# ctu-vras/depth_correction

Measured on AMD Instinct MI355X. Metric: points/sec through min_eigval_loss fwd+bwd (200k pts, k=10); HBM GB/s vs peak, higher is better.
Workload: dtype f64

## Files before the change

### depth_correction_amd/csrc/dc_cons_chain.h

```cpp
#pragma once

namespace dc {

struct AdamArgs {
  double* p; double* m; double* v;
  int n;
  double grad_scale, lr, b1, b2, eps, weight_decay, bias1, bias2_sqrt;
};
__device__ __forceinline__ void adam_apply(const AdamArgs& a, int i, double grad, double p0, double m0, double v0) {
  double g = grad * a.grad_scale;
  if (a.weight_decay != 0.0) g += a.weight_decay * p0;
  const double mi = m0 + (g - m0) * (1.0 - a.b1);
  const double vi = v0 * a.b2 + (1.0 - a.b2) * g * g;
  a.m[i] = mi; a.v[i] = vi;
  const double denom = sqrt(vi) / a.bias2_sqrt + a.eps;
  a.p[i] = p0 + (-(a.lr / a.bias1)) * (mi / denom);
}
__device__ __forceinline__ void adam_update(const AdamArgs& a, int i, double grad) { adam_apply(a, i, grad, a.p[i], a.m[i], a.v[i]); }

struct StepChain {
  int32_t* ready;
  uint32_t stamp;
  int parity, has_prev, n_front, n_out;
  int reverse;
  const double* prev;
  int64_t prev_rows;
  const double* grad_sum;
  double* out_prev;
  double* w_prev_out;
  int32_t* status;
  int spin_limit;
  const double* w_now;
  const int32_t* prev_status;
  const double* acc_in;
  AdamArgs adam;
  const uint8_t* blk_skip;
};
constexpr int32_t kStatusChainTimeout = 2;
constexpr int kChainFront = 8;

__device__ __forceinline__ int64_t chain_block_of(const StepChain& ch, bool chained, int64_t nblocks) {
  const int64_t b = (int64_t)blockIdx.x - (chained ? ch.n_front : 0);
  if (!(chained && ch.reverse)) return xcd_block_of(b, nblocks);
  const int64_t per = (nblocks + kXcds - 1) / kXcds;
  const int64_t logical = (b % kXcds) * per + (per - 1 - b / kXcds);
  return logical < nblocks ? logical : -1;
}

__device__ __forceinline__ void chain_publish(const StepChain& ch, int k, double w) {
  unsigned long long* pub = reinterpret_cast<unsigned long long*>(ch.ready);
  const unsigned long long st = (unsigned long long)ch.stamp << 32;
  __hip_atomic_store(pub + 2 * k, st | (unsigned)__double2loint(w), __ATOMIC_RELAXED, __HIP_MEMORY_SCOPE_AGENT);
  __hip_atomic_store(pub + 2 * k + 1, st | (unsigned)__double2hiint(w), __ATOMIC_RELAXED, __HIP_MEMORY_SCOPE_AGENT);
}

template <int P>
__device__ __forceinline__ void chain_front_block(const StepChain& ch, double* lds ) {
  const int a = blockIdx.x;
  if (a == 0 && ch.has_prev && !ch.grad_sum)
    for (int z = 2 + P + threadIdx.x; z < ch.n_out; z += kBlock) ch.out_prev[z] = 0.0;
  if (a >= 2 + P) return;
  if (ch.grad_sum) {
    if (a >= 2 && threadIdx.x == 0) {
      if (ch.has_prev && ch.adam.p) adam_update(ch.adam, a - 2, ch.grad_sum[a - 2]);
      const double wk = ch.adam.p ? ch.adam.p[a - 2] : ch.w_now[a - 2];
      chain_publish(ch, a - 2, wk);
      if (ch.w_prev_out) ch.w_prev_out[a - 2] = wk;
    }
    return;
  }
  const bool step = ch.has_prev && ch.adam.p && a >= 2 && threadIdx.x == 0;
  const int32_t* st_prev = ch.prev_status ? ch.prev_status : ch.status;
  const bool flagged = ch.has_prev && a == 0 && threadIdx.x == 0 && st_prev &&
                       __hip_atomic_load(st_prev, __ATOMIC_RELAXED, __HIP_MEMORY_SCOPE_AGENT) != 0;
  double p0 = 0.0, m0 = 0.0, v0 = 0.0;
  if (step) {
    p0 = ch.adam.p[a - 2]; m0 = ch.adam.m[a - 2]; v0 = ch.adam.v[a - 2];
    if (ch.w_prev_out) ch.w_prev_out[a - 2] = p0;
  }
  double s = 0.0;
  if (ch.has_prev) {
    const double* p = ch.prev + (int64_t)a * ch.prev_rows;
    constexpr int U = 32;
    for (int64_t r0 = threadIdx.x; r0 < ch.prev_rows; r0 += (int64_t)U * kBlock) {
      double v[U];
#pragma unroll
      for (int u_ = 0; u_ < U; ++u_) v[u_] = (r0 + (int64_t)u_ * kBlock < ch.prev_rows) ? p[r0 + (int64_t)u_ * kBlock] : 0.0;
#pragma unroll
      for (int w_ = U / 2; w_ > 0; w_ >>= 1) {
#pragma unroll
        for (int u_ = 0; u_ < w_; ++u_) v[u_] += v[u_ + w_];
      }
      s += v[0];
    }
    s = wave_sum(s);
  }
  const int lane = threadIdx.x & (kWave - 1), wave = threadIdx.x / kWave;
  if (lane == 0) lds[wave] = s;
  __syncthreads();
  if (threadIdx.x == 0) {
    if (ch.has_prev) {
      double t = 0.0;
      for (int wv = 0; wv < kBlock / kWave; ++wv) t += lds[wv];
      if (ch.acc_in) t += ch.acc_in[a];
      if (flagged) t = __longlong_as_double(0x7ff8000000000000ll);
      ch.out_prev[a] = t;
      if (step) adam_apply(ch.adam, a - 2, t, p0, m0, v0);
    }
    if (a >= 2) chain_publish(ch, a - 2, step ? ch.adam.p[a - 2] : ch.w_now[a - 2]);
  }
}

template <int P>
__global__ __launch_bounds__(kBlock) void chain_front_only_kernel(StepChain ch) {
  __shared__ double s_front[kBlock / kWave];
  chain_front_block<P>(ch, s_front);
}

template <int P>
__device__ __forceinline__ void chain_weights(const StepChain& ch, double w_scale, double* s_w, int* s_ok) {
  const int tid = threadIdx.x;
  if (tid == 0) *s_ok = 1;
  if (tid < 2 * P) {
    const unsigned long long* pub = reinterpret_cast<const unsigned long long*>(ch.ready) + tid;
    unsigned long long word = 0;
    bool ok = false;
    for (int spin = 0; spin < ch.spin_limit; ++spin) {
      word = __hip_atomic_load(pub, __ATOMIC_RELAXED, __HIP_MEMORY_SCOPE_AGENT);
      if ((uint32_t)(word >> 32) == ch.stamp) { ok = true; break; }
      __builtin_amdgcn_s_sleep(2);
    }
    const int half = (int)(uint32_t)word;
    const int other = __shfl_xor(half, 1, kWave);
    if ((tid & 1) == 0) s_w[tid >> 1] = (ok ? __hiloint2double(other, half) : __longlong_as_double(0x7ff8000000000000ll)) * w_scale;
    if (!ok) {
      *s_ok = 0;
      if (ch.status) atomicOr(ch.status, kStatusChainTimeout);
    }
  }
}

}
```

### depth_correction_amd/csrc/dc_cons_step.h

```cpp
#pragma once

namespace dc {

template <typename PT, int P> struct StepRow;
template <int P> struct StepRow<q32, P> {
  static constexpr int kPieces = (6 + P + 3) / 4;
  struct Raw { int32_t q[6 + P]; };
  static __device__ __forceinline__ Raw fetch(const PointBasis& pb, int64_t row) {
    const int32_t* r = static_cast<const int32_t*>(pb.rows) + row * (6 + P);
    Raw o;
#pragma unroll
    for (int c = 0; c < 6 + P; ++c) o.q[c] = r[c];
    return o;
  }
  static __device__ __forceinline__ void stage(const PointBasis& pb, const double* wq, int64_t row, int4* tile, int cap, int t) {
    place(fetch(pb, row), wq, tile, cap, t);
  }
  static __device__ __forceinline__ void place(const Raw& raw, const double* wq, int4* tile, int cap, int t) {
    const int32_t* q = raw.q;
    float sc = 0.0f;
#pragma unroll
    for (int k = 0; k < P; ++k) sc = fmaf((float)wq[k], __int_as_float(q[6 + k]), sc);
    int32_t x[3];
#pragma unroll
// ... 199 lines not shown
    for (int u_ = 0; u_ < kTrip; ++u_) nxt[u_] = (q0 + kTrip + u_ < nslots) ? (uint32_t)lrow[(q0 + kTrip + u_) * kBlock] : kNoLoc;
    float g[P];
#pragma unroll
    for (int k = 0; k < P; ++k) g[k] = 0.0f;
#pragma unroll
    for (int u_ = 0; u_ < kTrip; ++u_) chain_term_f32<P>(tile, cap, l[u_], l[u_] != kNoLoc, ci, cmf, vs, vu, c2f, g);
#pragma unroll
    for (int k = 0; k < P; ++k) gw[k] += (double)g[k];
  }
}
template <typename PT, int P>
__device__ __forceinline__ void chain_tail(const int4* tile, int cap, const uint16_t* lrow, int nslots, bool packed, const double* mean,
                                           const double* v0, double c1, double c2, double* gw) {
  uint32_t nxt[kTrip];
#pragma unroll
  for (int u_ = 0; u_ < kTrip; ++u_) nxt[u_] = (kPreSlots + u_ < nslots) ? (uint32_t)lrow[(kPreSlots + u_) * kBlock] : kNoLoc;
  for (int q0 = kPreSlots; q0 < nslots; q0 += kTrip) {
    uint32_t l[kTrip];
#pragma unroll
    for (int u_ = 0; u_ < kTrip; ++u_) l[u_] = nxt[u_];
    if (packed && __all((int)(l[0] == kNoLoc))) break;
#pragma unroll
    for (int u_ = 0; u_ < kTrip; ++u_) nxt[u_] = (q0 + kTrip + u_ < nslots) ? (uint32_t)lrow[(q0 + kTrip + u_) * kBlock] : kNoLoc;
#pragma unroll
    for (int u_ = 0; u_ < kTrip; ++u_) chain_term<PT, P>(tile, cap, l[u_], l[u_] != kNoLoc, mean, v0, c1, c2, gw);
  }
}

template <int CTRL>
__device__ __forceinline__ double dpp_f64(double v) {
  const int lo = __builtin_amdgcn_mov_dpp(__double2loint(v), CTRL, 0xF, 0xF, true);
  const int hi = __builtin_amdgcn_mov_dpp(__double2hiint(v), CTRL, 0xF, 0xF, true);
  return __hiloint2double(hi, lo);
}
constexpr int kDppXor1 = 0xB1;
constexpr int kDppXor2 = 0x4E;
constexpr int kDppRor4 = 0x124;
constexpr int kDppRor8 = 0x128;
constexpr int kDppShl4 = 0x104;
constexpr int kDppQuad3 = 0xFF;
__device__ __forceinline__ double wave_sum4_dpp(double* v) {
  const int lane = threadIdx.x & (kWave - 1);
  const bool up1 = (lane & 1) != 0, up2 = (lane & 2) != 0;
  const double k0 = up1 ? v[2] : v[0], g0 = up1 ? v[0] : v[2];
  const double k1 = up1 ? v[3] : v[1], g1 = up1 ? v[1] : v[3];
  const double a0 = k0 + dpp_f64<kDppXor1>(g0);
  const double a1 = k1 + dpp_f64<kDppXor1>(g1);
  const double kk = up2 ? a1 : a0, gg = up2 ? a0 : a1;
  double r = kk + dpp_f64<kDppXor2>(gg);
  r += dpp_f64<kDppRor4>(r);
  r += dpp_f64<kDppRor8>(r);
  r += __shfl_xor(r, 16, kWave);
  r += __shfl_xor(r, 32, kWave);
  return r;
}

template <int P, bool DPP = false>
__device__ __forceinline__ void step_partials(const double* acc2, const double* gw, double* __restrict__ p_fwd, double* __restrict__ p_bwd,
                                              bool per_block = false, int n_front = 0) {
  constexpr int NV = 2 + P, NP2 = NV <= 4 ? 4 : 8;
  __shared__ double s_comb[kWavesPerBlock][NP2];
  double v[NP2];
  v[0] = acc2[0]; v[1] = acc2[1];
#pragma unroll
  for (int k = 0; k < NP2 - 2; ++k) v[2 + k] = k < P ? gw[k] : 0.0;
  double tot;
  if constexpr (DPP && NP2 == 4) tot = wave_sum4_dpp(v);
  else tot = wave_sum_packed<NP2>(v);
  const int lane = threadIdx.x & (kWave - 1), wave = threadIdx.x / kWave;
  int64_t rs = (int64_t)gridDim.x * kWavesPerBlock, row = (int64_t)blockIdx.x * kWavesPerBlock + wave;
  if (per_block) {
    if (lane < NP2) s_comb[wave][lane] = tot;
    __syncthreads();
    if (wave != 0) return;
    if (lane < NP2) tot = (s_comb[0][lane] + s_comb[1][lane]) + (s_comb[2][lane] + s_comb[3][lane]);
    rs = (int64_t)gridDim.x - n_front;
    row = (int64_t)blockIdx.x - n_front;
  }
  if (lane < NP2) {
    const int q = packed_value_of_lane<NP2>(lane);
    if (q < 2) p_fwd[q * rs + row] = tot;
    else if (q < NV) p_bwd[(q - 2) * rs + row] = tot;
  }
}

template <typename PT, int NS, int P, int VAR = 0>
__global__ __launch_bounds__(kBlock) void consistency_step_basis_kernel(
    PointBasis pb, BlockTab tab, const int32_t* __restrict__ own_base, int cap, const int32_t* __restrict__ centre_idx, int64_t n,
    const uint8_t* __restrict__ mask, LossParams lp, QParams qp, double* __restrict__ p_fwd, double* __restrict__ p_bwd,
    StepChain ch) {
  extern __shared__ int4 tile[];
  __shared__ double s_w[DC_MAX_MODEL_TERMS];
  __shared__ int s_ok;
  __shared__ double s_front[kBlock / kWave];
  const bool chained = ch.ready != nullptr;
  if (chained && (int)blockIdx.x < ch.n_front) { chain_front_block<P>(ch, s_front); return; }
  const int64_t nblocks = (n + kBlock - 1) / kBlock;
  int64_t blk = chain_block_of(ch, chained, nblocks);
  if (blk >= 0 && ch.blk_skip && ch.blk_skip[blk]) blk = -1;
  double acc2[2] = {0.0, 0.0}, gw[P];
#pragma unroll
  for (int k = 0; k < P; ++k) gw[k] = 0.0;
  const int32_t s0 = blk >= 0 ? tab.slot_ptr[blk] : 0;
  bool bad = blk >= 0 && tab.slot_ptr[blk + 1] - s0 != NS;
  if (blk >= 0 && !bad) {
    const int64_t i = blk * kBlock + threadIdx.x;
// ... 64 lines not shown
            if (q % 4 == 0 && q > 0) __builtin_amdgcn_sched_barrier(0);
            chain_term_f32<P>(tile, cap, pre[q], true, ci, cmf, vs, vu, c2f, gwf);
          }
        }
#pragma unroll
        for (int k = 0; k < P; ++k) gw[k] = (double)gwf[k] * u;
      } else {
        double mean[3];
        StepRow<PT, P>::mean_of(ci, cm, mean);
        if (any_miss) {
#pragma unroll
          for (int q = 0; q < NS; ++q) chain_term<PT, P>(tile, cap, pre[q], pre[q] != kNoLoc, mean, v0, c1, c2, gw);
        } else {
#pragma unroll
          for (int q = 0; q < NS; ++q) chain_term<PT, P>(tile, cap, pre[q], true, mean, v0, c1, c2, gw);
        }
#pragma unroll
        for (int k = 0; k < P; ++k) gw[k] *= u;
      }
    }
  }
  if (bad) acc2[0] = acc2[1] = __longlong_as_double(0x7ff8000000000000ll);
  step_partials<P, (VAR & kVarDppSums) != 0>(acc2, gw, p_fwd, p_bwd, chained, chained ? ch.n_front : 0);
}

constexpr int kStepQ32Cap = 512;

typedef float float2v __attribute__((ext_vector_type(2)));
template <int P, int CAP>
__device__ __forceinline__ void chain_term_q32(const int4* tile, uint32_t off, bool have, const Pt<q32>::Raw& ci, const float* cmf, const float* vs,
                                               const float* vu, float c2f, float* gw) {
  const char* row = reinterpret_cast<const char*>(tile) + (have ? off : 0u);
  const int4 p0 = *reinterpret_cast<const int4*>(row);
  const int4 p1 = *reinterpret_cast<const int4*>(row + (size_t)CAP * 16);
  const float2v e01 = float2v{(float)(p0.x - ci.v[0]), (float)(p0.y - ci.v[1])} - float2v{cmf[0], cmf[1]};
  const float e0 = e01.x, e1 = e01.y, e2 = (float)(p0.z - ci.v[2]) - cmf[2];
  const float u0 = __int_as_float(p0.w), u1 = __int_as_float(p1.x), u2 = __int_as_float(p1.y);
  const float al = fmaf(vs[2], e2, fmaf(vs[1], e1, vs[0] * e0));
  const float be = fmaf(vu[2], u2, fmaf(vu[1], u1, vu[0] * u0));
  const float ga = fmaf(e2, u2, fmaf(e1, u1, e0 * u0));
  float tj = fmaf(al, be, -(c2f * ga));
  if (!have) tj = 0.0f;
  if constexpr (P == 2) {
    float2v g = float2v{gw[0], gw[1]};
    g = __builtin_elementwise_fma(float2v{tj, tj}, float2v{__int_as_float(p1.z), __int_as_float(p1.w)}, g);
    gw[0] = g.x; gw[1] = g.y;
  } else {
    gw[0] = fmaf(tj, __int_as_float(p1.z), gw[0]);
    if constexpr (P > 1) gw[1] = fmaf(tj, __int_as_float(p1.w), gw[1]);
    if constexpr (P > 2) gw[2] = fmaf(tj, __int_as_float(reinterpret_cast<const int4*>(row + (size_t)CAP * 32)->x), gw[2]);
  }
}

#ifdef DC_BLOCK_TRACE
__device__ unsigned long long* g_block_trace = nullptr;
#define DC_TRACE_BEGIN() const unsigned long long trace_t0 = __builtin_amdgcn_s_memrealtime()
#define DC_TRACE_END() do { if (threadIdx.x == 0 && g_block_trace) { \
    unsigned long long* tr_ = g_block_trace + 4 * (size_t)blockIdx.x; \
    tr_[0] = ((unsigned long long)__builtin_amdgcn_s_getreg((31 << 11) | 20) << 32) | (unsigned)__builtin_amdgcn_s_getreg((31 << 11) | 4); \
    tr_[1] = trace_t0; tr_[2] = __builtin_amdgcn_s_memrealtime(); tr_[3] = 1; } } while (0)
#else
#define DC_TRACE_BEGIN() do {} while (0)
#define DC_TRACE_END() do {} while (0)
#endif

template <int NS, int P, int CAP>
__global__ __launch_bounds__(kBlock, (StepRow<q32, P>::kPieces * CAP * 16 <= 25 * 1024 ? 6 : 4)) void consistency_step_q32_kernel(
    PointBasis pb, BlockTab tab, const int32_t* __restrict__ own_base, const int32_t* __restrict__ centre_idx, int64_t n,
    const uint8_t* __restrict__ mask, LossParams lp, QParams qp, double* __restrict__ p_fwd, double* __restrict__ p_bwd,
    StepChain ch) {
  constexpr int NV = 2 + P, NP2 = NV <= 4 ? 4 : 8;
  constexpr int cap = CAP;
  __shared__ int4 tile[StepRow<q32, P>::kPieces * CAP];
  __shared__ double s_w[DC_MAX_MODEL_TERMS];
  __shared__ double s_front[kWavesPerBlock];
  __shared__ double s_comb[kWavesPerBlock * NP2];
  __shared__ int s_ok[2];
  DC_TRACE_BEGIN();
  const bool chained = ch.ready != nullptr;
  if (chained && (int)blockIdx.x < ch.n_front) { chain_front_block<P>(ch, s_front); return; }
  const int64_t nblocks = (n + kBlock - 1) / kBlock;
  int64_t blk = chain_block_of(ch, chained, nblocks);
  if (blk >= 0 && ch.blk_skip && ch.blk_skip[blk]) blk = -1;
  double acc2[2] = {0.0, 0.0}, gw[P];
#pragma unroll
  for (int k = 0; k < P; ++k) gw[k] = 0.0;
  const int32_t s0 = blk >= 0 ? tab.slot_ptr[blk] : 0;
  bool bad = blk >= 0 && tab.slot_ptr[blk + 1] - s0 != NS;
  if (blk >= 0 && !bad) {
    const int64_t i = blk * kBlock + threadIdx.x;
    const bool live = i < n;
    const bool in_mask = live && (mask ? mask[i] != 0 : true);
    const uint16_t* lrow = tab.loc + (int64_t)s0 * kBlock + threadIdx.x;
    uint32_t pre[NS];
#pragma unroll
    for (int q = 0; q < NS; ++q) pre[q] = (uint32_t)lrow[q * kBlock];
    const int32_t base = tab.blk_ptr[blk], nd = tab.blk_ptr[blk + 1] - base;
    const int32_t own = (own_base && !centre_idx) ? own_base[blk] : -1;
    double wq[P];
    if (chained) {
      typename StepRow<q32, P>::Raw r0, r1;
      const int t0 = threadIdx.x, t1 = threadIdx.x + kBlock;
      if (t0 < nd) r0 = StepRow<q32, P>::fetch(pb, tab.blk_ids[base + t0]);
      if (t1 < nd) r1 = StepRow<q32, P>::fetch(pb, tab.blk_ids[base + t1]);
      chain_weights<P>(ch, pb.w_scale, s_w, s_ok);
      __syncthreads();
      if (!s_ok[0]) bad = true;
#pragma unroll
      for (int k = 0; k < P; ++k) wq[k] = s_w[k];
      if (t0 < nd) StepRow<q32, P>::place(r0, wq, tile, cap, t0);
      if (t1 < nd) StepRow<q32, P>::place(r1, wq, tile, cap, t1);
      for (int t = threadIdx.x + 2 * kBlock; t < nd; t += kBlock) StepRow<q32, P>::stage(pb, wq, tab.blk_ids[base + t], tile, cap, t);
    } else {
      stage_weights(pb, s_w);
      __syncthreads();
#pragma unroll
      for (int k = 0; k < P; ++k) wq[k] = s_w[k];
      for (int t = threadIdx.x; t < nd; t += kBlock) StepRow<q32, P>::stage(pb, wq, tab.blk_ids[base + t], tile, cap, t);
    }
    Pt<q32>::Raw ci;
    if (own < 0) ci = Basis<q32>::template point<P>(pb, wq, live ? (centre_idx ? (int64_t)centre_idx[i] : i) : 0);
    __syncthreads();
    if (own >= 0) ci = staged_point<q32>(tile, cap, own + (live ? (int)threadIdx.x : 0));
    if (live && (!mask || __any((int)in_mask))) {
      CovAcc acc;
      cov_init(acc);
      uint32_t mo = pre[0];
#pragma unroll
      for (int q = 1; q < NS; ++q) mo |= pre[q];
      const bool any_miss = __any((int)(mo & 1u)) != 0;
      int n_have;
      if (any_miss) n_have = gather_fixed<q32, NS, true>(tile, cap, ci, pre, acc);
      else n_have = gather_fixed<q32, NS, false>(tile, cap, ci, pre, acc);
      acc.W = (double)n_have;
      double cm[3], v0[3], c1, c2;
      step_point2<q32, NS>(acc, n_have, !any_miss, in_mask, lp, qp, acc2, cm, v0, &c1, &c2);
      float cmf[3], vs[3], vu[3], gwf[P];
#pragma unroll
      for (int a = 0; a < 3; ++a) { cmf[a] = (float)cm[a]; vs[a] = (float)(c1 * v0[a]); vu[a] = (float)v0[a]; }
      const float c2f = (float)c2;
#pragma unroll
      for (int k = 0; k < P; ++k) gwf[k] = 0.0f;
      if (any_miss) {
#pragma unroll
        for (int q = 0; q < NS; ++q) {
          if (q % 4 == 0 && q > 0) __builtin_amdgcn_sched_barrier(0);
          chain_term_q32<P, CAP>(tile, pre[q], pre[q] != kNoLoc, ci, cmf, vs, vu, c2f, gwf);
        }
      } else {
#pragma unroll
        for (int q = 0; q < NS; ++q) {
          if (q % 4 == 0 && q > 0) __builtin_amdgcn_sched_barrier(0);
          chain_term_q32<P, CAP>(tile, pre[q], true, ci, cmf, vs, vu, c2f, gwf);
        }
      }
      const double u = qp.scale;
#pragma unroll
      for (int k = 0; k < P; ++k) gw[k] = (double)gwf[k] * u;
    }
  }
  if (bad) acc2[0] = acc2[1] = __longlong_as_double(0x7ff8000000000000ll);
  double v[NP2];
  v[0] = acc2[0]; v[1] = acc2[1];
#pragma unroll
  for (int k = 0; k < NP2 - 2; ++k) v[2 + k] = k < P ? gw[k] : 0.0;
  double tot;
  if constexpr (NP2 == 4) tot = wave_sum4_dpp(v);
  else tot = wave_sum_packed<NP2>(v);
  const int lane = threadIdx.x & (kWave - 1), wave = threadIdx.x / kWave;
  int64_t rs = (int64_t)gridDim.x * kWavesPerBlock, row = (int64_t)blockIdx.x * kWavesPerBlock + wave;
  if (chained) {
    if (lane < NP2) s_comb[wave * NP2 + lane] = tot;
    __syncthreads();
    if (wave != 0) return;
    if (lane < NP2) tot = (s_comb[lane] + s_comb[NP2 + lane]) + (s_comb[2 * NP2 + lane] + s_comb[3 * NP2 + lane]);
    rs = (int64_t)gridDim.x - ch.n_front;
    row = (int64_t)blockIdx.x - ch.n_front;
  }
  if (lane < NP2) {
    const int q = packed_value_of_lane<NP2>(lane);
    if (q < 2) p_fwd[q * rs + row] = tot;
    else if (q < NV) p_bwd[(q - 2) * rs + row] = tot;
  }
  DC_TRACE_END();
}

template <typename PT, int P>
__global__ __launch_bounds__(kBlock) void consistency_step_basis_slots_kernel(
    PointBasis pb, BlockTab tab, const int32_t* __restrict__ own_base, int cap, const int32_t* __restrict__ centre_idx, int64_t n,
    const uint8_t* __restrict__ mask, LossParams lp, QParams qp, double* __restrict__ p_fwd, double* __restrict__ p_bwd,
    StepChain ch, int packed) {
  extern __shared__ int4 tile[];
  __shared__ double s_w[DC_MAX_MODEL_TERMS];
  __shared__ int s_ok;
  __shared__ double s_front[kBlock / kWave];
  const bool chained = ch.ready != nullptr;
  if (chained && (int)blockIdx.x < ch.n_front) { chain_front_block<P>(ch, s_front); return; }
  const int64_t nblocks = (n + kBlock - 1) / kBlock;
  int64_t blk = xcd_block_of((int64_t)blockIdx.x - (chained ? ch.n_front : 0), nblocks);
  if (blk >= 0 && ch.blk_skip && ch.blk_skip[blk]) blk = -1;
  double acc2[2] = {0.0, 0.0}, gw[P];
#pragma unroll
  for (int k = 0; k < P; ++k) gw[k] = 0.0;
  const int64_t i = blk * kBlock + threadIdx.x;
  const bool live = blk >= 0 && i < n;
  int32_t nslots = 0, own = -1, base = 0, nd = 0;
  const uint16_t* lrow = tab.loc;
  uint32_t pre[kPreSlots];
  if (blk >= 0) {
    const int32_t s0 = tab.slot_ptr[blk];
    nslots = tab.slot_ptr[blk + 1] - s0;
    lrow = tab.loc + (int64_t)s0 * kBlock + threadIdx.x;
#pragma unroll
    for (int q = 0; q < kPreSlots; ++q) pre[q] = (live && q < nslots) ? (uint32_t)lrow[q * kBlock] : kNoLoc;
    own = (own_base && !centre_idx) ? own_base[blk] : -1;
    base = tab.blk_ptr[blk];
    nd = tab.blk_ptr[blk + 1] - base;
  }
  double wq[P];
  bool timed_out = false;
  typename Pt<PT>::Raw ci;
  if (chained) {
// ... 222 lines not shown
```

### depth_correction_amd/csrc/dc_consistency.hip

```cpp
#include <type_traits>
#include <atomic>
#include <mutex>
#include <cstdio>
#include <hip/hip_ext.h>
#include "dc_common.h"
#include "dc_device.h"
#include "dc_pointmath.h"
#include "dc_prof.h"
#include "dc_points_dev.h"
#include "../../include/dc_hip.h"

namespace dc {

template <typename T, typename PT, int STRIDE>
__global__ __launch_bounds__(kBlock) void points_fwd_kernel(PointInputs in, int64_t n, QParams qp, PT* __restrict__ x_out,
                                                            T* __restrict__ vps_out, T* __restrict__ dirs_out,
                                                            T* __restrict__ depth_out) {
  __shared__ double s_pose[kLdsScans * 12];
  const int64_t i = (int64_t)blockIdx.x * kBlock + threadIdx.x;
  const int64_t ic = i < n ? i : n - 1;
  ModelParams mp;
  load_model(in, mp);
  T vp_r[3] = {T(0), T(0), T(0)}, dr_r[3];
  if (in.vps) { const T* q = (const T*)in.vps + ic * 3; vp_r[0] = q[0]; vp_r[1] = q[1]; vp_r[2] = q[2]; }
// ... 943 lines not shown
  const bool step = adam.p && a >= 2 && a - 2 < adam.n && threadIdx.x == 0;
  double p0 = 0.0, m0 = 0.0, v0 = 0.0;
  if (step) { p0 = adam.p[a - 2]; m0 = adam.m[a - 2]; v0 = adam.v[a - 2]; }
  const double s = wave_sum(strided_sum(p, n_rows));
  if (lane == 0) lds[wave] = s;
  __syncthreads();
  if (threadIdx.x == 0) {
    double t = 0.0;
    for (int wv = 0; wv < kRedBlock / kWave; ++wv) t += lds[wv];
    if (flagged) t = __longlong_as_double(0x7ff8000000000000ll);
    out[a] = t;
    if (step) adam_apply(adam, a - 2, t, p0, m0, v0);
  }
}

static inline unsigned red_grid(int n_red, int pose_first, int pose_cols) {
  if (pose_first < 0 || n_red <= pose_first) return 2u + (unsigned)n_red;
  return 2u + (unsigned)pose_first + (unsigned)((pose_cols + kPoseRedCols - 1) / kPoseRedCols);
}

__global__ void adam_kernel(const double* __restrict__ grad, AdamArgs adam) {
  const int i = (int)(blockIdx.x * blockDim.x + threadIdx.x);
  if (i < adam.n) adam_update(adam, i, grad[i]);
}

__global__ __launch_bounds__(256) void adam_device_step_kernel(const double* __restrict__ grad, AdamArgs adam, int64_t* __restrict__ step) {
  const double t = (double)(*step + 1);
  adam.bias1 = 1.0 - pow(adam.b1, t);
  adam.bias2_sqrt = sqrt(1.0 - pow(adam.b2, t));
  for (int i = threadIdx.x; i < adam.n; i += blockDim.x) adam_update(adam, i, grad[i]);
  __syncthreads();
  if (threadIdx.x == 0) *step = (int64_t)t;
}

}

using namespace dc;

#define DC_CHECK_LAUNCH()                                  \
  do {                                                     \
    hipError_t err__ = hipGetLastError();                  \
    if (err__ != hipSuccess) return (int)err__;            \
  } while (0)

static inline int64_t n_blocks(int64_t n) { return (n + kBlock - 1) / kBlock; }
static std::atomic<bool> g_no_tab{false};
static std::atomic<int> g_fwd_generic{0};
static std::atomic<bool> g_no_basis{false};
static std::atomic<bool> g_two_pass{false};
static std::atomic<int> g_chain_spin{1 << 22};
static std::atomic<int> g_step_var{1};
static std::atomic<bool> g_pose_three_pass{false};
static std::atomic<bool> g_no_reverse{false};

template <int P, int CAP>
static int ragged_launch(dim3 grid, hipStream_t stream, hipEvent_t ev0, hipEvent_t ev1, const PointBasis& pb, const BlockTab& tab,
                         const dcBlockTable* t, int64_t n_rows, const uint8_t* mask, const LossParams& lp, const QParams& qp, double* p_fwd,
                         double* p_bwd, const StepChain& ch) {
  constexpr size_t bytes = (size_t)StepRow<q32, P>::kPieces * CAP * 16;
  static std::atomic<uint64_t> attr_set{0};
  if (bytes > 60 * 1024) {
    int dev = 0;
    if (hipGetDevice(&dev) != hipSuccess) dev = 0;
    const uint64_t bit = 1ull << (dev & 63);
    if (!(attr_set.fetch_or(bit) & bit)) {
      hipError_t err = hipFuncSetAttribute((const void*)consistency_step_ragged_q32_kernel<P, CAP>, hipFuncAttributeMaxDynamicSharedMemorySize, (int)bytes);
      if (err != hipSuccess) { attr_set.fetch_and(~bit); return (int)err; }
    }
  }
  hipExtLaunchKernelGGL((consistency_step_ragged_q32_kernel<P, CAP>), grid, dim3(kBlock), bytes, stream, ev0, ev1, 0, pb, tab, t->own_base, t->row_ptr, n_rows,
                        mask, lp, qp, p_fwd, p_bwd, ch);
  return DC_OK;
}

static bool use_table(const dcBlockTable* t, int layout, int stride, uint32_t row_bytes, int extra_rows, size_t lds_limit,
                      size_t* lds_bytes, int* lds_rows) {
  if (!t || g_no_tab.load() || stride != 4 || t->layout != layout || !t->blk_ptr || !t->loc || t->max_rows < 0) return false;
  if (layout == DC_TABLE_SLOTS ? !t->slot_ptr : !t->run_ptr) return false;
  if (t->max_rows > 0 && !t->blk_ids) return false;
  const size_t rows = (size_t)t->max_rows + extra_rows + (t->max_rows + extra_rows == 0 ? 1 : 0);
  const size_t need = rows * row_bytes;
  if (need > lds_limit || t->max_rows >= 0xFFF) return false;
  *lds_bytes = need;
  *lds_rows = (int)rows;
  return true;
}

extern "C" {

int dc_version(void) { return 100; }

int64_t dc_partial_rows(int64_t n) { return xcd_grid(n_blocks(n)) * kWavesPerBlock; }

int dc_param_grad_count(int n_terms, int n_scans) { return 2 * n_terms + 12 * n_scans; }

int64_t dc_sequence_partials_count(int64_t n, int n_terms, int n_scans) {
  if (n < 0 || n_terms < 0 || n_scans < 0) return 0;
  const int64_t rows = xcd_grid(n_blocks(n)) * kWavesPerBlock;
  return rows * (2 + 2 * (int64_t)n_terms + 12 * (int64_t)n_scans) + 2 * (2 + (int64_t)n_terms) * rows;
}

static PointInputs make_inputs(const void* vps, const void* dirs, const void* depth, const void* inc,
                               const uint8_t* lmask, const int32_t* scan_id, const double* poses, int n_scans,
                               int model_kind, int n_terms, const double* w, const double* e) {
  PointInputs in;
  in.vps = vps; in.dirs = dirs; in.depth = depth; in.inc = inc; in.lmask = lmask; in.scan_id = scan_id;
// ... 295 lines not shown
  if (n < 0 || !grad_points || !dirs || !depth || !partials_ws || !grads_out || (stride != 3 && stride != 4))
    return DC_ERR_ARG;
  if (scan_id && (!poses || n_scans < 1)) return DC_ERR_ARG;
  int rc = check_model(model_kind, n_terms, inc, w, e);
  if (rc) return rc;
  if (model_kind == DC_MODEL_NONE) n_terms = 0;
  const int n_acc = 2 * n_terms + 12 * n_scans;
  if (n_acc == 0) return DC_OK;
  if (n == 0) return (int)hipMemsetAsync(grads_out, 0, n_acc * sizeof(double), stream);
  PointInputs in = make_inputs(vps, dirs, depth, inc, lmask, scan_id, poses, n_scans, model_kind, n_terms, w, e);
  const int64_t rows = n_blocks(n);
  const int64_t prows = rows * kWavesPerBlock;
  dim3 grid((unsigned)rows), block(kBlock);
  const int n_red = want_pose_grad ? n_acc : 2 * n_terms;
  if (n_red < n_acc) {
    hipError_t err = hipMemsetAsync(grads_out + n_red, 0, (size_t)(n_acc - n_red) * sizeof(double), stream);
    if (err != hipSuccess) return (int)err;
  }
  if (n_red == 0) return DC_OK;
  if (want_pose_grad) {
    hipError_t err = hipMemsetAsync(partials_ws + (size_t)prows * 2 * n_terms, 0, (size_t)prows * 12 * n_scans * sizeof(double), stream);
    if (err != hipSuccess) return (int)err;
  }
#define LAUNCH(T, S) \
  hipLaunchKernelGGL((points_bwd_kernel<T, S>), grid, block, 0, stream, (const T*)grad_points, perm, n, in, \
                     want_exponent_grad, want_pose_grad, partials_ws, n_acc)
  if (dtype == DC_F32) { if (stride == 3) LAUNCH(float, 3); else LAUNCH(float, 4); }
  else if (dtype == DC_F64) { if (stride == 3) LAUNCH(double, 3); else LAUNCH(double, 4); }
  else return DC_ERR_DTYPE;
#undef LAUNCH
  DC_CHECK_LAUNCH();
  hipLaunchKernelGGL(reduce_partials_kernel, dim3(n_red), dim3(kRedBlock), 0, stream, partials_ws, prows, grads_out);
  DC_CHECK_LAUNCH();
  return DC_OK;
}

#ifdef DC_BLOCK_TRACE
int dc_debug_block_trace(void* buf) {
  unsigned long long* p = (unsigned long long*)buf;
  return (int)hipMemcpyToSymbol(HIP_SYMBOL(dc::g_block_trace), &p, sizeof(p));
}
#endif
int dc_set_option(int option, int value) {
  static const bool enabled = [] { const char* e = getenv("DC_ENABLE_ABLATIONS"); return e && atoi(e) != 0; }();
  if (!enabled) return DC_ERR_UNSUPPORTED;
  if (option == 0) { g_no_tab.store(value != 0); return DC_OK; }
  if (option == 1) { g_fwd_generic.store(value); return DC_OK; }
  if (option == 3) { g_no_basis.store(value != 0); return DC_OK; }
  if (option == 4) { g_two_pass.store(value != 0); return DC_OK; }
  if (option == 5) { g_chain_spin.store(value < 0 ? (1 << 22) : value); return DC_OK; }
  if (option == 6) { g_step_var.store(value); return DC_OK; }
  if (option == 7) { g_pose_three_pass.store(value != 0); return DC_OK; }
  if (option == 8) { g_no_reverse.store(value != 0); return DC_OK; }
  return DC_ERR_ARG;
}

int dc_profiler_enable(int every) {
  std::lock_guard<std::mutex> lock(g_prof.mu);
  g_prof.every = every < 0 ? 0 : every;
  return DC_OK;
}
int dc_profiler_reset(void) {
  std::lock_guard<std::mutex> lock(g_prof.mu);
  for (int k = 0; k < kProfKinds; ++k) { g_prof.count[k] = 0; g_prof.seen[k] = 0; }
  return DC_OK;
}
int dc_profiler_kernel(int kind, char* buf, int len) {
  if (kind < 0 || kind >= kProfKinds || !buf || len < 1) return DC_ERR_ARG;
  const char* nm = g_prof.last_kernel[kind];
  snprintf(buf, (size_t)len, "%s", nm ? nm : "");
  return DC_OK;
}
int dc_profiler_read(int kind, double* total_ms, int64_t* launches) {
  if (kind < 0 || kind >= kProfKinds || !total_ms || !launches) return DC_ERR_ARG;
  double tot = 0.0;
  int n;
  { std::lock_guard<std::mutex> lock(g_prof.mu); n = g_prof.count[kind]; }
  for (int i = 0; i < n; ++i) {
    hipError_t err = hipEventSynchronize(g_prof.stop[kind][i]);
    if (err != hipSuccess) return (int)err;
    float ms = 0.f;
    err = hipEventElapsedTime(&ms, g_prof.start[kind][i], g_prof.stop[kind][i]);
    if (err != hipSuccess) return (int)err;
    tot += ms;
  }
  *total_ms = tot;
  *launches = n;
  return DC_OK;
}

static int make_adam(double* param, double* exp_avg, double* exp_avg_sq, int64_t n, int64_t step, double grad_scale, double lr,
                     double beta1, double beta2, double eps, double weight_decay, AdamArgs* a) {
  if (!param || !exp_avg || !exp_avg_sq || n < 0 || n > 0x7fffffff || step < 1) return DC_ERR_ARG;
  *a = AdamArgs{param, exp_avg, exp_avg_sq, (int)n, grad_scale, lr, beta1, beta2, eps, weight_decay,
                1.0 - pow(beta1, (double)step), sqrt(1.0 - pow(beta2, (double)step))};
  return DC_OK;
}

int dc_adam_step(double* param, const double* grad, double* exp_avg, double* exp_avg_sq, int64_t n, int64_t step,
                 double grad_scale, double lr, double beta1, double beta2, double eps, double weight_decay,
                 hipStream_t stream) {
  AdamArgs a;
  int rc = make_adam(param, exp_avg, exp_avg_sq, n, step, grad_scale, lr, beta1, beta2, eps, weight_decay, &a);
  if (rc || !grad) return rc ? rc : DC_ERR_ARG;
  if (n == 0) return DC_OK;
  hipLaunchKernelGGL(adam_kernel, dim3((unsigned)((n + 63) / 64)), dim3(64), 0, stream, grad, a);
// ... 86 lines not shown
  const bool basis = basis_fwd &&
                     (!want_grad || one_pass || use_table(d->bwd_table, DC_TABLE_RUNS, stride, q32_pts ? 32u : 64u, 1, 44 * 1024, &lds_b, &rows_b));
  const int fixed_k = g_fwd_generic.load() ? 0 : d->k;
  if ((chain || one_pass_only) && !(basis && one_pass)) return DC_ERR_UNSUPPORTED;
  if (basis) {
    QParams qp;
    int rc = make_qparams(d->point_fmt, d->dtype, stride, d->qparams, &qp);
    if (rc) return rc;
    PointBasis pb{d->basis, w, n_terms, q32_pts ? qp.inv_scale : 1.0};
    const LossParams lp = make_loss_params(d->loss_kind & ~DC_LOSS_RAW_POINTWISE, d->normalization, d->sqrt_);
    BlockTab tab{d->fwd_table->blk_ptr, d->fwd_table->blk_ids, d->fwd_table->slot_ptr, d->fwd_table->loc};
    const dim3 block(kBlock);
    if (one_pass) {
      const int64_t g_blocks = xcd_grid(n_blocks(n_rows));
      StepChain ch{};
      ch.blk_skip = (d->mask && !d->centre_idx) ? d->blk_skip : nullptr;
      if (chain) {
        p_fwd = chain_buffer(d, n_terms, chain->parity);
        p_bwd = p_fwd + 2 * g_blocks;
        ch.ready = chain->ready; ch.parity = chain->parity; ch.has_prev = chain->has_prev; ch.n_front = kChainFront;
        ch.n_out = 2 + n_acc; ch.prev = chain_buffer(d, n_terms, chain->parity ^ 1); ch.prev_rows = g_blocks;
        if (chain->prev_rows) { ch.prev = chain->prev_rows; ch.prev_rows = chain->prev_count; }
        ch.acc_in = chain->acc_in; ch.prev_status = chain->prev_status;
        ch.out_prev = chain->out_prev; ch.w_prev_out = chain->w_prev_out; ch.status = d->status; ch.spin_limit = g_chain_spin.load(); ch.adam = chain->adam_prev;
        ch.grad_sum = chain->grad_sum;
        ch.stamp = chain->stamp; ch.w_now = w;
        ch.reverse = (chain->parity && !g_no_reverse.load()) ? 1 : 0;
      }
      const dim3 grid((unsigned)(g_blocks + (chain ? kChainFront : 0)));
      const int var = g_step_var.load();
      const bool q32_step = q32_pts && var == 1 && (fixed_k == 10 || fixed_k == 4 || fixed_k == 8 || fixed_k == 16) && rows_s <= 768;
      const bool ragged_step = ragged_ok;
      if (ragged_step) {
        ProfScope prof(1);
        const int mr = rag_rows;
        int rc = DC_OK;
#define RAGGED(P, CAP) (prof.name("(consistency_step_ragged_q32_kernel<" #P ", " #CAP ">)"), \
                        ragged_launch<P, CAP>(grid, stream, prof.start(), prof.stop(), pb, tab, d->fwd_table, n_rows, d->mask, lp, qp, p_fwd, p_bwd, ch))
#define RAGGED_CAPS(P) (mr <= 1024 ? RAGGED(P, 1024) : mr <= 1280 ? RAGGED(P, 1280) : mr <= 1600 ? RAGGED(P, 1600) : mr <= 2048 ? RAGGED(P, 2048) : \
                        mr <= 2560 ? RAGGED(P, 2560) : RAGGED(P, 4096))
        if (n_terms == 2) rc = RAGGED_CAPS(2);
        else if (n_terms == 1) rc = RAGGED_CAPS(1);
        else rc = mr <= 1024 ? RAGGED(3, 1024) : mr <= 1600 ? RAGGED(3, 1600) : RAGGED(3, 2560);
#undef RAGGED_CAPS
#undef RAGGED
        if (rc) return rc;
      } else if (q32_step) {
        ProfScope prof(1);
        static_assert(kStepQ32Cap == 512, "the profiler names the instantiation by its literal arguments");
#define STEPQ_LAUNCH(NS, P, CAP) DC_TIMED_LAUNCH((consistency_step_q32_kernel<NS, P, CAP>), grid, block, 0, stream, pb, tab, d->fwd_table->own_base, \
                                                 d->centre_idx, n_rows, d->mask, lp, qp, p_fwd, p_bwd, ch)
#define STEPQ_P(NS, CAP) do { if (n_terms == 2) STEPQ_LAUNCH(NS, 2, CAP); else if (n_terms == 1) STEPQ_LAUNCH(NS, 1, CAP); else STEPQ_LAUNCH(NS, 3, CAP); } while (0)
#define STEPQ_K(CAP) do { if (fixed_k == 10) STEPQ_P(10, CAP); else if (fixed_k == 4) STEPQ_P(4, CAP); else if (fixed_k == 8) STEPQ_P(8, CAP); else STEPQ_P(16, CAP); } while (0)
        if (rows_s <= 512) STEPQ_K(512); else STEPQ_K(768);
#undef STEPQ_K
#undef STEPQ_P
#undef STEPQ_LAUNCH
      } else {
        ProfScope prof(1);
#define STEP_LAUNCH(K) DC_TIMED_LAUNCH(K, grid, block, lds_s, stream, pb, tab, d->fwd_table->own_base, rows_s, d->centre_idx, n_rows, \
                                       d->mask, lp, qp, p_fwd, p_bwd, ch)
#define STEP_NS(PT, P) do { if (fixed_k == 10 && P == 2 && var == 0) STEP_LAUNCH((consistency_step_basis_kernel<PT, 10, 2, 0>)); \
                            else if (fixed_k == 10) STEP_LAUNCH((consistency_step_basis_kernel<PT, 10, P, kStepVar>)); \
                            else if (fixed_k == 4) STEP_LAUNCH((consistency_step_basis_kernel<PT, 4, P, kStepVar>)); \
                            else if (fixed_k == 8) STEP_LAUNCH((consistency_step_basis_kernel<PT, 8, P, kStepVar>)); \
                            else if (fixed_k == 16) STEP_LAUNCH((consistency_step_basis_kernel<PT, 16, P, kStepVar>)); \
                            else DC_TIMED_LAUNCH((consistency_step_basis_slots_kernel<PT, P>), grid, block, lds_s, stream, pb, tab, d->fwd_table->own_base, rows_s, \
                                                 d->centre_idx, n_rows, d->mask, lp, qp, p_fwd, p_bwd, ch, d->fwd_table->packed); } while (0)
#define STEP(PT) do { if (n_terms == 2) STEP_NS(PT, 2); else if (n_terms == 1) STEP_NS(PT, 1); else STEP_NS(PT, 3); } while (0)
        if (q32_pts) STEP(q32); else STEP(double);
#undef STEP
#undef STEP_NS
#undef STEP_LAUNCH
      }
      DC_CHECK_LAUNCH();
      if (chain && chain->reduce_now) {
        hipLaunchKernelGGL(reduce_eval_kernel, dim3(2 + n_terms), dim3(kRedBlock), 0, stream, p_fwd, p_bwd, g_blocks, g_blocks, n_terms,
                           2 + n_acc, out, AdamArgs{}, (const int32_t*)d->status);
        DC_CHECK_LAUNCH();
      }
      if (chain) return DC_OK;
      const int64_t rows_g = (int64_t)grid.x * kWavesPerBlock;
      hipLaunchKernelGGL(reduce_eval_kernel, dim3(2 + n_terms), dim3(kRedBlock), 0, stream, p_fwd, p_bwd, rows_g, rows_g, n_terms, 2 + n_acc, out,
                         adam, (const int32_t*)d->status);
      DC_CHECK_LAUNCH();
      return DC_OK;
    }
    {
      ProfScope prof(1);
      const dim3 grid((unsigned)xcd_grid(n_blocks(n_rows)));
#define FWD_BASIS_P(PT, T, NS, P) DC_TIMED_LAUNCH((consistency_fwd_basis_kernel<PT, false, NS, P>), grid, block, lds_f, stream, pb, tab, \
                                                 d->fwd_table->own_base, rows_f, d->centre_idx, n_rows, d->mask, (const T*)nullptr, lp, qp, \
                                                 (PT*)(want_grad ? d->rec : nullptr), (T*)nullptr, (T*)nullptr, p_fwd)
#define FWD_BASIS_SLOTS(PT, T, P) DC_TIMED_LAUNCH((consistency_fwd_basis_slots_kernel<PT, false, P>), grid, block, lds_f, stream, pb, tab, \
                                                 d->fwd_table->own_base, rows_f, d->centre_idx, n_rows, d->mask, (const T*)nullptr, lp, qp, \
                                                 (PT*)(want_grad ? d->rec : nullptr), (T*)nullptr, (T*)nullptr, p_fwd)
#define FWD_BASIS_NS(PT, T, P) do { if (fixed_k == 10) FWD_BASIS_P(PT, T, 10, P); else if (fixed_k == 4) FWD_BASIS_P(PT, T, 4, P); \
                                    else if (fixed_k == 8) FWD_BASIS_P(PT, T, 8, P); else if (fixed_k == 16) FWD_BASIS_P(PT, T, 16, P); \
                                    else FWD_BASIS_SLOTS(PT, T, P); } while (0)
#define FWD_BASIS(PT, T) do { if (n_terms == 2) FWD_BASIS_NS(PT, T, 2); else if (n_terms == 1) FWD_BASIS_NS(PT, T, 1); \
                              else if (n_terms == 3) FWD_BASIS_NS(PT, T, 3); else FWD_BASIS_NS(PT, T, 0); } while (0)
      if (q32_pts) FWD_BASIS(q32, float); else FWD_BASIS(double, double);
#undef FWD_BASIS
#undef FWD_BASIS_NS
#undef FWD_BASIS_SLOTS
#undef FWD_BASIS_P
    }
// ... 217 lines not shown
```

Before: 52.23 billion.

## Pack neighbour offsets, raise step kernel occupancy, ballot-count loss terms

The q32 consistency step kernel now packs the 16-bit neighbour locations two per register and gathers through new packed helpers. Launch bounds are derived from the LDS footprint so the kernel can reach 7 blocks per CU, and the count term is computed with a ballot and popcount instead of being wave-summed. An 8-wide register shuffle reduction replaces the packed wave sum, and the chain front block spreads its Adam state loads across three lanes and reads them back with readlane. The centre point is re-materialised before the backward sweep to shorten register live ranges, and an option-gated six-block variant is added. The aim is lower register pressure and higher occupancy, at the risk of spills or slower gathers.

```diff
diff --git a/depth_correction_amd/csrc/dc_cons_chain.h b/depth_correction_amd/csrc/dc_cons_chain.h
--- a/depth_correction_amd/csrc/dc_cons_chain.h
+++ b/depth_correction_amd/csrc/dc_cons_chain.h
@@ -54,6 +54,10 @@
   __hip_atomic_store(pub + 2 * k + 1, st | (unsigned)__double2hiint(w), __ATOMIC_RELAXED, __HIP_MEMORY_SCOPE_AGENT);
 }
 
+__device__ __forceinline__ double lane_value_f64(double v, int l) {
+  return __hiloint2double(__builtin_amdgcn_readlane(__double2hiint(v), l), __builtin_amdgcn_readlane(__double2loint(v), l));
+}
+
 template <int P>
 __device__ __forceinline__ void chain_front_block(const StepChain& ch, double* lds ) {
   const int a = blockIdx.x;
@@ -69,23 +73,28 @@
     }
     return;
   }
-  const bool step = ch.has_prev && ch.adam.p && a >= 2 && threadIdx.x == 0;
+  const bool step_blk = ch.has_prev && ch.adam.p && a >= 2;
+  const bool step = step_blk && threadIdx.x == 0;
   const int32_t* st_prev = ch.prev_status ? ch.prev_status : ch.status;
   const bool flagged = ch.has_prev && a == 0 && threadIdx.x == 0 && st_prev &&
                        __hip_atomic_load(st_prev, __ATOMIC_RELAXED, __HIP_MEMORY_SCOPE_AGENT) != 0;
-  double p0 = 0.0, m0 = 0.0, v0 = 0.0;
-  if (step) {
-    p0 = ch.adam.p[a - 2]; m0 = ch.adam.m[a - 2]; v0 = ch.adam.v[a - 2];
-    if (ch.w_prev_out) ch.w_prev_out[a - 2] = p0;
+  double st = 0.0;
+  if (step_blk && threadIdx.x < 3) {
+    const double* src = threadIdx.x == 0 ? ch.adam.p : threadIdx.x == 1 ? ch.adam.m : ch.adam.v;
+    st = src[a - 2];
+    if (threadIdx.x == 0 && ch.w_prev_out) ch.w_prev_out[a - 2] = st;
   }
   double s = 0.0;
   if (ch.has_prev) {
-    const double* p = ch.prev + (int64_t)a * ch.prev_rows;
     constexpr int U = 32;
-    for (int64_t r0 = threadIdx.x; r0 < ch.prev_rows; r0 += (int64_t)U * kBlock) {
+    const int64_t rows = ch.prev_rows;
+    const uint32_t tid = threadIdx.x;
+    for (int64_t b0 = 0; b0 < rows; b0 += (int64_t)U * kBlock) {
+      const double* p = ch.prev + (int64_t)a * rows + b0;
+      const uint32_t left = rows - b0 < (int64_t)U * kBlock ? (uint32_t)(rows - b0) : (uint32_t)(U * kBlock);
       double v[U];
 #pragma unroll
-      for (int u_ = 0; u_ < U; ++u_) v[u_] = (r0 + (int64_t)u_ * kBlock < ch.prev_rows) ? p[r0 + (int64_t)u_ * kBlock] : 0.0;
+      for (int u_ = 0; u_ < U; ++u_) v[u_] = (tid + (uint32_t)(u_ * kBlock) < left) ? p[tid + (uint32_t)(u_ * kBlock)] : 0.0;
 #pragma unroll
       for (int w_ = U / 2; w_ > 0; w_ >>= 1) {
 #pragma unroll
@@ -98,6 +107,7 @@
   const int lane = threadIdx.x & (kWave - 1), wave = threadIdx.x / kWave;
   if (lane == 0) lds[wave] = s;
   __syncthreads();
+  const double p0 = lane_value_f64(st, 0), m0 = lane_value_f64(st, 1), v0 = lane_value_f64(st, 2);
   if (threadIdx.x == 0) {
     if (ch.has_prev) {
       double t = 0.0;
diff --git a/depth_correction_amd/csrc/dc_cons_step.h b/depth_correction_amd/csrc/dc_cons_step.h
--- a/depth_correction_amd/csrc/dc_cons_step.h
+++ b/depth_correction_amd/csrc/dc_cons_step.h
@@ -275,6 +275,27 @@
   r += dpp_f64<kDppRor8>(r);
   r += __shfl_xor(r, 16, kWave);
   r += __shfl_xor(r, 32, kWave);
+  return r;
+}
+
+__device__ __forceinline__ double wave_sum8_regs(const double* v) {
+  const int lane = threadIdx.x & (kWave - 1);
+  const bool up1 = (lane & 1) != 0, up2 = (lane & 2) != 0, up4 = (lane & 4) != 0;
+  double a[4], b[2];
+#pragma unroll
+  for (int k = 0; k < 4; ++k) {
+    const double keep = up1 ? v[k + 4] : v[k], give = up1 ? v[k] : v[k + 4];
+    a[k] = keep + __shfl_xor(give, 1, kWave);
+  }
+#pragma unroll
+  for (int k = 0; k < 2; ++k) {
+    const double keep = up2 ? a[k + 2] : a[k], give = up2 ? a[k] : a[k + 2];
+    b[k] = keep + __shfl_xor(give, 2, kWave);
+  }
+  const double keep = up4 ? b[1] : b[0], give = up4 ? b[0] : b[1];
+  double r = keep + __shfl_xor(give, 4, kWave);
+#pragma unroll
+  for (int off = 8; off < kWave; off <<= 1) r += __shfl_xor(r, off, kWave);
   return r;
 }
 
@@ -445,6 +466,51 @@
   }
 }
 
+template <int P, int CAP> constexpr int step_q32_blocks() {
+  constexpr int lds = StepRow<q32, P>::kPieces * CAP * 16 + 512;
+  return 7 * lds <= 160 * 1024 ? 7 : 6 * lds <= 160 * 1024 ? 6 : 4;
+}
+template <int Q> __device__ __forceinline__ uint32_t pre_at(const uint32_t* pk) { return (Q & 1) ? pk[Q >> 1] >> 16 : pk[Q >> 1] & 0xFFFFu; }
+template <int NS, bool MISS, int Q0 = 0>
+__device__ __forceinline__ int gather_fixed_pk(const int4* tile, const Pt<q32>::Raw& ci, const uint32_t* pk, CovAcc& acc) {
+  if constexpr (Q0 >= NS) return 0;
+  else {
+    constexpr int NQ = NS - Q0 < 4 ? NS - Q0 : 4;
+    uint32_t off[NQ];
+    off[0] = pre_at<Q0>(pk);
+    if constexpr (NQ > 1) off[1] = pre_at<Q0 + (NQ > 1 ? 1 : 0)>(pk);
+    if constexpr (NQ > 2) off[2] = pre_at<Q0 + (NQ > 2 ? 2 : 0)>(pk);
+    if constexpr (NQ > 3) off[3] = pre_at<Q0 + (NQ > 3 ? 3 : 0)>(pk);
+    Pt<q32>::Raw cj[NQ];
+    bool have[NQ];
+    int n_have = 0;
+#pragma unroll
+    for (int u_ = 0; u_ < NQ; ++u_) {
+      have[u_] = !MISS || off[u_] != kNoLoc;
+      int4 piece[1];
+      read_row<1>(tile, 0, have[u_] ? off[u_] : 0u, piece);
+      cj[u_] = Pt<q32>::from_row(piece);
+    }
+#pragma unroll
+    for (int u_ = 0; u_ < NQ; ++u_) {
+      double d[3];
+      Pt<q32>::delta(have[u_] ? cj[u_] : ci, ci, d);
+      cov_add_d(acc, d[0], d[1], d[2]);
+      n_have += have[u_] ? 1 : 0;
+    }
+    return n_have + gather_fixed_pk<NS, MISS, Q0 + 4>(tile, ci, pk, acc);
+  }
+}
+template <int NS, int P, int CAP, bool MISS, int Q = 0>
+__device__ __forceinline__ void chain_sweep_pk(const int4* tile, const uint32_t* pk, const Pt<q32>::Raw& ci, const float* cmf, const float* vs,
+                                               const float* vu, float c2f, float* gwf) {
+  if constexpr (Q < NS) {
+    if constexpr (Q % 4 == 0 && Q > 0) __builtin_amdgcn_sched_barrier(0);
+    const uint32_t off = pre_at<Q>(pk);
+    chain_term_q32<P, CAP>(tile, off, !MISS || off != kNoLoc, ci, cmf, vs, vu, c2f, gwf);
+    chain_sweep_pk<NS, P, CAP, MISS, Q + 1>(tile, pk, ci, cmf, vs, vu, c2f, gwf);
+  }
+}
 #ifdef DC_BLOCK_TRACE
 __device__ unsigned long long* g_block_trace = nullptr;
 #define DC_TRACE_BEGIN() const unsigned long long trace_t0 = __builtin_amdgcn_s_memrealtime()
@@ -457,8 +523,8 @@
 #define DC_TRACE_END() do {} while (0)
 #endif
 
-template <int NS, int P, int CAP>
-__global__ __launch_bounds__(kBlock, (StepRow<q32, P>::kPieces * CAP * 16 <= 25 * 1024 ? 6 : 4)) void consistency_step_q32_kernel(
+template <int NS, int P, int CAP, int BLOCKS = step_q32_blocks<P, CAP>()>
+__global__ __launch_bounds__(kBlock, BLOCKS) void consistency_step_q32_kernel(
     PointBasis pb, BlockTab tab, const int32_t* __restrict__ own_base, const int32_t* __restrict__ centre_idx, int64_t n,
     const uint8_t* __restrict__ mask, LossParams lp, QParams qp, double* __restrict__ p_fwd, double* __restrict__ p_bwd,
     StepChain ch) {
@@ -475,27 +541,35 @@
   const int64_t nblocks = (n + kBlock - 1) / kBlock;
   int64_t blk = chain_block_of(ch, chained, nblocks);
   if (blk >= 0 && ch.blk_skip && ch.blk_skip[blk]) blk = -1;
-  double acc2[2] = {0.0, 0.0}, gw[P];
+  double loss = 0.0, gw[P];
+  bool cnt_lane = false;
 #pragma unroll
   for (int k = 0; k < P; ++k) gw[k] = 0.0;
   const int32_t s0 = blk >= 0 ? tab.slot_ptr[blk] : 0;
   bool bad = blk >= 0 && tab.slot_ptr[blk + 1] - s0 != NS;
   if (blk >= 0 && !bad) {
-    const int64_t i = blk * kBlock + threadIdx.x;
-    const bool live = i < n;
-    const bool in_mask = live && (mask ? mask[i] != 0 : true);
-    const uint16_t* lrow = tab.loc + (int64_t)s0 * kBlock + threadIdx.x;
-    uint32_t pre[NS];
-#pragma unroll
-    for (int q = 0; q < NS; ++q) pre[q] = (uint32_t)lrow[q * kBlock];
+    const uint32_t tid = threadIdx.x;
+    const int64_t i0 = blk * kBlock, left = n - i0;
+    const uint32_t n_live = left < kBlock ? (uint32_t)left : (uint32_t)kBlock;
+    const bool live = tid < n_live;
+    const uint8_t* mask_blk = mask ? mask + i0 : nullptr;
+    const bool in_mask = live && (mask_blk ? mask_blk[tid] != 0 : true);
+    const uint16_t* lrow = tab.loc + (int64_t)s0 * kBlock;
+    constexpr int NW = (NS + 1) / 2;
+    uint32_t pk[NW];
+#pragma unroll
+    for (int j = 0; j < NW; ++j)
+      pk[j] = (uint32_t)lrow[(uint32_t)(2 * j * kBlock) + tid] |
+              (2 * j + 1 < NS ? (uint32_t)lrow[(uint32_t)((2 * j + 1 < NS ? 2 * j + 1 : 0) * kBlock) + tid] << 16 : 0u);
     const int32_t base = tab.blk_ptr[blk], nd = tab.blk_ptr[blk + 1] - base;
     const int32_t own = (own_base && !centre_idx) ? own_base[blk] : -1;
+    const int32_t* ids = tab.blk_ids + base;
     double wq[P];
     if (chained) {
       typename StepRow<q32, P>::Raw r0, r1;
-      const int t0 = threadIdx.x, t1 = threadIdx.x + kBlock;
-      if (t0 < nd) r0 = StepRow<q32, P>::fetch(pb, tab.blk_ids[base + t0]);
-      if (t1 < nd) r1 = StepRow<q32, P>::fetch(pb, tab.blk_ids[base + t1]);
+      const int t0 = (int)tid, t1 = (int)tid + kBlock;
+      if (t0 < nd) r0 = StepRow<q32, P>::fetch(pb, ids[t0]);
+      if (t1 < nd) r1 = StepRow<q32, P>::fetch(pb, ids[t1]);
       chain_weights<P>(ch, pb.w_scale, s_w, s_ok);
       __syncthreads();
       if (!s_ok[0]) bad = true;
@@ -503,64 +577,68 @@
       for (int k = 0; k < P; ++k) wq[k] = s_w[k];
       if (t0 < nd) StepRow<q32, P>::place(r0, wq, tile, cap, t0);
       if (t1 < nd) StepRow<q32, P>::place(r1, wq, tile, cap, t1);
-      for (int t = threadIdx.x + 2 * kBlock; t < nd; t += kBlock) StepRow<q32, P>::stage(pb, wq, tab.blk_ids[base + t], tile, cap, t);
+      for (int t = (int)tid + 2 * kBlock; t < nd; t += kBlock) StepRow<q32, P>::stage(pb, wq, ids[t], tile, cap, t);
     } else {
       stage_weights(pb, s_w);
       __syncthreads();
 #pragma unroll
       for (int k = 0; k < P; ++k) wq[k] = s_w[k];
-      for (int t = threadIdx.x; t < nd; t += kBlock) StepRow<q32, P>::stage(pb, wq, tab.blk_ids[base + t], tile, cap, t);
+      for (int t = (int)tid; t < nd; t += kBlock) StepRow<q32, P>::stage(pb, wq, ids[t], tile, cap, t);
     }
     Pt<q32>::Raw ci;
-    if (own < 0) ci = Basis<q32>::template point<P>(pb, wq, live ? (centre_idx ? (int64_t)centre_idx[i] : i) : 0);
+    if (own < 0) ci = Basis<q32>::template point<P>(pb, wq, live ? (centre_idx ? (int64_t)(centre_idx + i0)[tid] : i0 + tid) : 0);
     __syncthreads();
-    if (own >= 0) ci = staged_point<q32>(tile, cap, own + (live ? (int)threadIdx.x : 0));
+    if (own >= 0) ci = staged_point<q32>(tile, cap, own + (live ? (int)tid : 0));
     if (live && (!mask || __any((int)in_mask))) {
       CovAcc acc;
       cov_init(acc);
-      uint32_t mo = pre[0];
-#pragma unroll
-      for (int q = 1; q < NS; ++q) mo |= pre[q];
-      const bool any_miss = __any((int)(mo & 1u)) != 0;
+      uint32_t mo = pk[0];
+#pragma unroll
+      for (int j = 1; j < NW; ++j) mo |= pk[j];
+      const bool any_miss = __any((int)(mo & 0x00010001u)) != 0;
       int n_have;
-      if (any_miss) n_have = gather_fixed<q32, NS, true>(tile, cap, ci, pre, acc);
-      else n_have = gather_fixed<q32, NS, false>(tile, cap, ci, pre, acc);
+      if (any_miss) n_have = gather_fixed_pk<NS, true>(tile, ci, pk, acc);
+      else n_have = gather_fixed_pk<NS, false>(tile, ci, pk, acc);
       acc.W = (double)n_have;
-      double cm[3], v0[3], c1, c2;
+      double cm[3], v0[3], c1, c2, acc2[2] = {0.0, 0.0};
       step_point2<q32, NS>(acc, n_have, !any_miss, in_mask, lp, qp, acc2, cm, v0, &c1, &c2);
+      loss = acc2[0];
+      cnt_lane = acc2[1] != 0.0;
       float cmf[3], vs[3], vu[3], gwf[P];
 #pragma unroll
       for (int a = 0; a < 3; ++a) { cmf[a] = (float)cm[a]; vs[a] = (float)(c1 * v0[a]); vu[a] = (float)v0[a]; }
       const float c2f = (float)c2;
 #pragma unroll
       for (int k = 0; k < P; ++k) gwf[k] = 0.0f;
-      if (any_miss) {
-#pragma unroll
-        for (int q = 0; q < NS; ++q) {
-          if (q % 4 == 0 && q > 0) __builtin_amdgcn_sched_barrier(0);
-          chain_term_q32<P, CAP>(tile, pre[q], pre[q] != kNoLoc, ci, cmf, vs, vu, c2f, gwf);
-        }
+      asm volatile("" ::: "memory");
+      Pt<q32>::Raw cs;
+      if (own >= 0) {
+        cs = staged_point<q32>(tile, cap, own + (int)tid);
       } else {
-#pragma unroll
-        for (int q = 0; q < NS; ++q) {
-          if (q % 4 == 0 && q > 0) __builtin_amdgcn_sched_barrier(0);
-          chain_term_q32<P, CAP>(tile, pre[q], true, ci, cmf, vs, vu, c2f, gwf);
-        }
+        double w2[P];
+#pragma unroll
+        for (int k = 0; k < P; ++k) w2[k] = s_w[k];
+        cs = Basis<q32>::template point<P>(pb, w2, centre_idx ? (int64_t)(centre_idx + i0)[tid] : i0 + tid);
       }
+      if (any_miss) chain_sweep_pk<NS, P, CAP, true>(tile, pk, cs, cmf, vs, vu, c2f, gwf);
+      else chain_sweep_pk<NS, P, CAP, false>(tile, pk, cs, cmf, vs, vu, c2f, gwf);
       const double u = qp.scale;
 #pragma unroll
       for (int k = 0; k < P; ++k) gw[k] = (double)gwf[k] * u;
     }
   }
-  if (bad) acc2[0] = acc2[1] = __longlong_as_double(0x7ff8000000000000ll);
+  const double nan_ = __longlong_as_double(0x7ff8000000000000ll);
+  if (bad) loss = nan_;
+  const double cnt = bad ? nan_ : (double)__popcll(__ballot((int)cnt_lane));
   double v[NP2];
-  v[0] = acc2[0]; v[1] = acc2[1];
+  v[0] = loss; v[1] = 0.0;
 #pragma unroll
   for (int k = 0; k < NP2 - 2; ++k) v[2 + k] = k < P ? gw[k] : 0.0;
   double tot;
   if constexpr (NP2 == 4) tot = wave_sum4_dpp(v);
-  else tot = wave_sum_packed<NP2>(v);
+  else tot = wave_sum8_regs(v);
   const int lane = threadIdx.x & (kWave - 1), wave = threadIdx.x / kWave;
+  if (packed_value_of_lane<NP2>(lane & (NP2 - 1)) == 1) tot = cnt;
   int64_t rs = (int64_t)gridDim.x * kWavesPerBlock, row = (int64_t)blockIdx.x * kWavesPerBlock + wave;
   if (chained) {
     if (lane < NP2) s_comb[wave * NP2 + lane] = tot;
diff --git a/depth_correction_amd/csrc/dc_consistency.hip b/depth_correction_amd/csrc/dc_consistency.hip
--- a/depth_correction_amd/csrc/dc_consistency.hip
+++ b/depth_correction_amd/csrc/dc_consistency.hip
@@ -1019,6 +1019,7 @@
 static std::atomic<int> g_step_var{1};
 static std::atomic<bool> g_pose_three_pass{false};
 static std::atomic<bool> g_no_reverse{false};
+static std::atomic<bool> g_step_six{false};
 
 template <int P, int CAP>
 static int ragged_launch(dim3 grid, hipStream_t stream, hipEvent_t ev0, hipEvent_t ev1, const PointBasis& pb, const BlockTab& tab,
@@ -1420,6 +1421,7 @@
   if (option == 6) { g_step_var.store(value); return DC_OK; }
   if (option == 7) { g_pose_three_pass.store(value != 0); return DC_OK; }
   if (option == 8) { g_no_reverse.store(value != 0); return DC_OK; }
+  if (option == 9) { g_step_six.store(value != 0); return DC_OK; }
   return DC_ERR_ARG;
 }
 
@@ -1612,7 +1614,16 @@
                                                  d->centre_idx, n_rows, d->mask, lp, qp, p_fwd, p_bwd, ch)
 #define STEPQ_P(NS, CAP) do { if (n_terms == 2) STEPQ_LAUNCH(NS, 2, CAP); else if (n_terms == 1) STEPQ_LAUNCH(NS, 1, CAP); else STEPQ_LAUNCH(NS, 3, CAP); } while (0)
 #define STEPQ_K(CAP) do { if (fixed_k == 10) STEPQ_P(10, CAP); else if (fixed_k == 4) STEPQ_P(4, CAP); else if (fixed_k == 8) STEPQ_P(8, CAP); else STEPQ_P(16, CAP); } while (0)
-        if (rows_s <= 512) STEPQ_K(512); else STEPQ_K(768);
+#define STEPQ_SIX(NS, P) DC_TIMED_LAUNCH((consistency_step_q32_kernel<NS, P, 512, 6>), grid, block, 0, stream, pb, tab, d->fwd_table->own_base, \
+                                         d->centre_idx, n_rows, d->mask, lp, qp, p_fwd, p_bwd, ch)
+#define STEPQ_SIX_P(NS) do { if (n_terms == 2) STEPQ_SIX(NS, 2); else STEPQ_SIX(NS, 1); } while (0)
+        static_assert(step_q32_blocks<1, 512>() == 7 && step_q32_blocks<2, 512>() == 7 && step_q32_blocks<3, 512>() == 6 && step_q32_blocks<2, 768>() == 6,
+                      "which instantiations dc_set_option(9, 1) has a six-block build of");
+        if (rows_s <= 512 && n_terms <= 2 && g_step_six.load()) {
+          if (fixed_k == 10) STEPQ_SIX_P(10); else if (fixed_k == 4) STEPQ_SIX_P(4); else if (fixed_k == 8) STEPQ_SIX_P(8); else STEPQ_SIX_P(16);
+        } else if (rows_s <= 512) STEPQ_K(512); else STEPQ_K(768);
+#undef STEPQ_SIX_P
+#undef STEPQ_SIX
 #undef STEPQ_K
 #undef STEPQ_P
 #undef STEPQ_LAUNCH
```

Result: faster. 54.32 billion, median of 6 (+4.0%).
